# ReadAlongs/SoundSwallower

Hardware: AMD Instinct MI355X
Metric: senone-frames/sec (en-us PTM) (higher is better)
Workload: dtype f32+i32

## Files before the change

soundswallower_amd/csrc/ssw_k1a_mfma.inc:

```
typedef _Float16 f16x8 __attribute__((ext_vector_type(8)));
typedef _Float16 f16x2 __attribute__((ext_vector_type(2)));

#define SSW_MFMA_WIDEN 1.8537045e-05f
#define SSW_MFMA_XMAX 255.0f

typedef uint32_t u32x4 __attribute__((ext_vector_type(4)));

struct SplitX {
    f16x8 p[2];
};

__device__ __forceinline__ SplitX
split2_f16(const float (&v)[8])
{
    SplitX s;
    float r[8];
#pragma unroll
    for (int j = 0; j < 8; ++j)
        r[j] = v[j];
#pragma unroll
    for (int p = 0; p < 2; ++p) {
        u32x4 w;
#pragma unroll
        for (int j = 0; j < 8; j += 2) {
            const float2v pr = { r[j], r[j + 1] };
            const f16x2 h = __builtin_convertvector(pr, f16x2);
            w[j >> 1] = __builtin_bit_cast(uint32_t, h);
            if (p == 0) {
                asm("v_fma_mix_f32 %0, %1, -1.0, %2 op_sel_hi:[1,0,0]"
                    : "=v"(r[j]) : "v"(w[j >> 1]), "v"(r[j]));
                asm("v_fma_mix_f32 %0, %1, -1.0, %2 op_sel:[1,0,0] op_sel_hi:[1,0,0]"
                    : "=v"(r[j + 1]) : "v"(w[j >> 1]), "v"(r[j + 1]));
            }
        }
        s.p[p] = __builtin_bit_cast(f16x8, w);
    }
    return s;
}

struct XRaw {
    float4u a, b;
};

template <int VECLEN>
__device__ __forceinline__ XRaw
mfma_load_x(const float *__restrict__ xp, bool hi)
{
    static_assert(VECLEN == 13, "K layout: 13 dimensions, the constant at slot 15");
    XRaw r;
    r.a = *reinterpret_cast<const float4u *>(xp + (hi ? 8 : 0));
    r.b = *reinterpret_cast<const float4u *>(xp + (hi ? 9 : 4));
    return r;
}

__device__ __forceinline__ void
mfma_build_x(const XRaw &r, bool hi, float xconst, SplitX (&bx)[2])
{
    const float4u a = r.a, b = r.b;
    float v0[8], v1[8];
    v0[0] = a.x, v0[1] = a.y, v0[2] = a.z, v0[3] = a.w;
    v0[4] = hi ? b.w : b.x;
    v0[5] = hi ? 32768.0f : b.y;
    v0[6] = hi ? 32768.0f : b.z;
    v0[7] = hi ? xconst : b.w;
#pragma unroll
    for (int j = 0; j < 5; ++j)
        v1[j] = v0[j] * v0[j];
    v1[5] = hi ? 0.0f : b.y * b.y;
    v1[6] = hi ? 0.0f : b.z * b.z;
    v1[7] = hi ? 0.0f : b.w * b.w;
    bx[0] = split2_f16(v0);
    bx[1] = split2_f16(v1);
}

template <int VECLEN>
__device__ __forceinline__ void
mfma_build_x(const float *__restrict__ xp, bool hi, float xconst, SplitX (&bx)[2])
{
    mfma_build_x(mfma_load_x<VECLEN>(xp, hi), hi, xconst, bx);
}

__device__ __forceinline__ v16f
mfma_key_tile_frag(const f16x8 (&a)[2][2], const SplitX (&bx)[2])
{
    v16f acc = {};
#pragma unroll
    for (int kb = 0; kb < 2; ++kb) {
        acc = __builtin_amdgcn_mfma_f32_32x32x16_f16(a[kb][0], bx[kb].p[1], acc, 0, 0, 0);
        acc = __builtin_amdgcn_mfma_f32_32x32x16_f16(a[kb][1], bx[kb].p[0], acc, 0, 0, 0);
    }
#pragma unroll
    for (int kb = 0; kb < 2; ++kb)
        acc = __builtin_amdgcn_mfma_f32_32x32x16_f16(a[kb][0], bx[kb].p[0], acc, 0, 0, 0);
    return acc;
}

__device__ __forceinline__ v16f
mfma_key_tile(const uint4 *s_w, int rb, int lane, const SplitX (&bx)[2])
{
    f16x8 a[2][2];
#pragma unroll
    for (int kb = 0; kb < 2; ++kb)
#pragma unroll
        for (int p = 0; p < 2; ++p)
            a[kb][p] = __builtin_bit_cast(f16x8, s_w[((rb * 2 + kb) * 2 + p) * 64 + lane]);
    return mfma_key_tile_frag(a, bx);
}

template <int VECLEN>
__global__ void __launch_bounds__(64)
ptm_mfma_keys_kernel(const uint4 *__restrict__ wfrag, const float *__restrict__ recmax,
                     const float *__restrict__ feats, int n_frames, int featdim, int foff, int cbf,
                     float *__restrict__ out)
{
    const int lane = threadIdx.x & 63, col = lane & 31;
    const bool hi = lane >= 32;
    __shared__ uint4 s_w[16 * 64];
    for (int i = lane; i < 16 * 64; i += 64)
        s_w[i] = wfrag[(size_t)cbf * (16 * 64) + i];
    const float scale = recmax[(size_t)cbf * SSW_REC_FLOATS + 1];
    const float xconst = recmax[(size_t)cbf * SSW_REC_FLOATS + 3];
    __syncthreads();
    for (int cb = 0; cb < 4; ++cb) {
        const int t = (int)blockIdx.x * 128 + 32 * cb + col;
        const int tl = t < n_frames ? t : n_frames - 1;
        const float *xp = feats + (size_t)tl * featdim + foff;
        SplitX bx[2];
        mfma_build_x<VECLEN>(xp, hi, xconst, bx);
        for (int rb = 0; rb < 4; ++rb) {
            const v16f acc = mfma_key_tile(s_w, rb, lane, bx);
            if (t < n_frames)
#pragma unroll
                for (int r = 0; r < 16; ++r)
                    out[(size_t)t * 128 + 32 * rb + 8 * (r >> 2) + (hi ? 4 : 0) + (r & 3)]
                        = acc[r] * scale;
        }
    }
}

#define SSW_TOP5_INSERT(L, key) ssw_top5_insert(L, key);

__device__ __forceinline__ void
mfma_label_keys(const v16f &acc, int rb, uint32_t keymask, float (&key)[16])
{
#pragma unroll
    for (int r = 0; r < 16; ++r) {
        uint32_t lab;
        asm("s_add_i32 %0, %1, %2" : "=s"(lab) : "s"(16 * rb), "i"(r) : "scc");
        key[r] = __uint_as_float((__float_as_uint(acc[r]) & keymask) | lab);
    }
}

__device__ __forceinline__ void
mfma_swap_merge(float (&LA)[5], const float (&LB)[5], bool hi, float (&L)[5])
{
    const uint32_t half_bit = hi ? 64u : 0u;
#pragma unroll
    for (int k = 0; k < 5; ++k) {
        const float mine = hi ? LB[k] : LA[k], send = hi ? LA[k] : LB[k];
        const float got = __shfl_xor(__uint_as_float(__float_as_uint(send) | half_bit), 32, WAVE);
        L[k] = __uint_as_float(__float_as_uint(mine) | half_bit);
        LA[k] = got;
    }
#pragma unroll
    for (int k = 0; k < 5; ++k)
        SSW_TOP5_INSERT(L, LA[k])
}

__device__ __forceinline__ uint32_t
mfma_label_density(uint32_t lab)
{
    return ((lab >> 4) & 3u) * 32u + ((lab >> 2) & 3u) * 8u + (lab >> 6) * 4u + (lab & 3u);
}

#ifndef SSW_MFMA_WAVES
#define SSW_MFMA_WAVES 5
#endif
template <int VECLEN, bool MS, int NSTEP, bool AUDIT = false, bool MASKED = false>
__global__ void __launch_bounds__(256, SSW_MFMA_WAVES)
ptm_topn_mfma_kernel(const float *__restrict__ rec, const uint4 *__restrict__ wfrag,
                     const float *__restrict__ recmax, const uint32_t *__restrict__ exlist,
                     const float *__restrict__ feats, FramesParams P)
{
    static_assert(VECLEN == 13, "K layout: 13 dimensions, the constant at slot 15");
    const int lane = threadIdx.x & 63;
    const int col = lane & 31;
    const bool hi = lane >= 32;
    const int pair = P.xcd_lo[blockIdx.x & 7u] + (int)(blockIdx.x >> 3);
    if (pair >= P.xcd_lo[(blockIdx.x & 7u) + 1])
        return;
    const int cbf = pair / P.tile_groups;
    const int tile = (pair - cbf * P.tile_groups) * 4
        + __builtin_amdgcn_readfirstlane((int)(threadIdx.x >> 6));
    const int t_base = P.frame_lo + tile * (64 * NSTEP);
    const int f = cbf % P.n_feat;
    const int foff = P.featoff[f];

    __shared__ float4 s_rec[128 * (SSW_REC28_FLOATS / 4)];
    __shared__ uint4 s_w[16 * 64];
    uint2 ustart_v[NSTEP];
#pragma unroll
    for (int q = 0; q < NSTEP; ++q) {
        const int tq = t_base + 64 * q < P.n_frames ? t_base + 64 * q : 0;
        ustart_v[q] = *reinterpret_cast<const uint2 *>(P.utt_start + (tq >> 5));
    }
    const float4 cbc = *reinterpret_cast<const float4 *>(recmax + (size_t)cbf * SSW_REC_FLOATS);
    const float d0 = cbc.x, scale = cbc.y, inv_scale = cbc.z, xconst = cbc.w;
    static_assert(SSW_EXLIST_STRIDE >= 129, "two entries per lane behind the count");
    const uint32_t *xl = exlist + (size_t)cbf * SSW_EXLIST_STRIDE;
    const uint32_t n_ex_v = xl[0], my_ex0 = xl[1 + lane], my_ex1 = xl[65 + lane];
    int n_ex;
    constexpr bool pre_x = NSTEP == 1;
    SplitX bxa[2], bxb[2];
    auto x_row = [&](int t) {
        return feats + (size_t)(t < P.n_frames ? t : P.n_frames - 1) * P.featdim + foff;
    };
    {
        const float4 *src = reinterpret_cast<const float4 *>(rec + (size_t)cbf * 128 * SSW_REC28_FLOATS);
        const uint4 *wsrc = wfrag + (size_t)cbf * (16 * 64);
        uint4 wst[4];
        float4 stage[4];
#pragma unroll
        for (int i = 0; i < 4; ++i)
            stage[i] = src[i * 256 + (int)threadIdx.x < 896 ? i * 256 + (int)threadIdx.x : 895];
#pragma unroll
        for (int i = 0; i < 4; ++i)
            wst[i] = wsrc[i * 256 + (int)threadIdx.x];
        XRaw ra, rb;
        if (pre_x) {
            ra = mfma_load_x<VECLEN>(x_row(t_base + col), hi);
            rb = mfma_load_x<VECLEN>(x_row(t_base + 32 + col), hi);
        }
#pragma unroll
        for (int i = 0; i < 4; ++i) {
            const int e = i * 256 + (int)threadIdx.x;
            if (e < 896)
                s_rec[e] = stage[i];
        }
#pragma unroll
        for (int i = 0; i < 4; ++i)
            s_w[i * 256 + (int)threadIdx.x] = wst[i];
        if (pre_x) {
            mfma_build_x(ra, hi, xconst, bxa);
            mfma_build_x(rb, hi, xconst, bxb);
        }
        n_ex = __builtin_amdgcn_readfirstlane((int)n_ex_v);
    }
    unsigned long long ustart[NSTEP];
#pragma unroll
    for (int q = 0; q < NSTEP; ++q)
        ustart[q] = ((unsigned long long)(uint32_t)__builtin_amdgcn_readfirstlane((int)ustart_v[q].y) << 32)
            | (uint32_t)__builtin_amdgcn_readfirstlane((int)ustart_v[q].x);
    __syncthreads();
    if (t_base >= P.n_frames)
        return;
    SSW_TL(0)
#ifdef SSW_TIMELINE
    if (lane == 0) {
        int wv = blockIdx.x * 4 + (threadIdx.x >> 6);
        if (wv < 8192) {
            g_timeline[wv * 6 + 4] = __builtin_amdgcn_s_getreg(63492);
            g_timeline[wv * 6 + 5] = __builtin_amdgcn_s_getreg(20 | (31 << 11));
        }
    }
#endif

    uint32_t keymask;
    asm volatile("v_mov_b32 %0, 0xffffff80" : "=v"(keymask));
    const float NEG_INF = -__builtin_huge_valf();
    const float *srec_f = reinterpret_cast<const float *>(s_rec);

    uint32_t cpk[2] = { 0u, 0u };
    int s3[2] = { 0, 0 };
    unsigned long long need[2] = { 0ull, 0ull };
    unsigned long long audited[2] = { 0ull, 0ull };
    const bool audit_wave = AUDIT && P.audit_k > 0
        && (pair * 4 + __builtin_amdgcn_readfirstlane((int)(threadIdx.x >> 6))) % P.audit_k == 0;

#pragma unroll 1
    for (int step = 0; step < NSTEP; ++step) {
        const int t0 = t_base + 64 * step;
        if (!pre_x) {
            mfma_build_x<VECLEN>(x_row(t0 + col), hi, xconst, bxa);
            mfma_build_x<VECLEN>(x_row(t0 + 32 + col), hi, xconst, bxb);
        }
        float LA[5], LB[5], MA[2], MB[2], ZA, ZB;
        ssw_top5_reset(LA, MA, ZA, NEG_INF);
        ssw_top5_reset(LB, MB, ZB, NEG_INF);
#pragma unroll 1
        for (int rb = 0; rb < 4; ++rb) {
            f16x8 a[2][2];
#pragma unroll
            for (int kb = 0; kb < 2; ++kb)
#pragma unroll
                for (int p = 0; p < 2; ++p)
                    a[kb][p] = __builtin_bit_cast(f16x8, s_w[((rb * 2 + kb) * 2 + p) * 64 + lane]);
            {
                const v16f acc = mfma_key_tile_frag(a, bxa);
                float key[16];
                mfma_label_keys(acc, rb, keymask, key);
                ssw_top5_tile(LA, MA, ZA, key);
            }
            {
                const v16f acc = mfma_key_tile_frag(a, bxb);
                float key[16];
                mfma_label_keys(acc, rb, keymask, key);
                ssw_top5_tile(LB, MB, ZB, key);
            }
        }
        ssw_top5_fold(LA, MA, ZA);
        ssw_top5_fold(LB, MB, ZB);
        float L[5];
        mfma_swap_merge(LA, LB, hi, L);
        const int t = t0 + lane;
        const int tl = t < P.n_frames ? t : P.n_frames - 1;
        const float *xp = feats + (size_t)tl * P.featdim + foff;
        float x[VECLEN];
#pragma unroll
        for (int j = 0; j + 4 <= VECLEN; j += 4) {
            const float4u v = *reinterpret_cast<const float4u *>(xp + j);
            x[j] = v.x, x[j + 1] = v.y, x[j + 2] = v.z, x[j + 3] = v.w;
        }
#pragma unroll
        for (int j = VECLEN & ~3; j < VECLEN; ++j)
            x[j] = xp[j];
        float2v x2[6];
#pragma unroll
        for (int p = 0; p < 6; ++p)
            x2[p] = float2v{ x[2 * p], x[2 * p + 1] };
        auto exact_row = [&](uint32_t row) -> float {
            const unsigned char *rowp = reinterpret_cast<const unsigned char *>(s_rec)
                + row * (SSW_REC28_FLOATS * 4);
            float4v rv[SSW_REC28_FLOATS / 4];
#pragma unroll
            for (int q = 0; q < SSW_REC28_FLOATS / 4; ++q)
                rv[q] = *reinterpret_cast<const float4v *>(rowp + q * 16);
            asm volatile("" : "+v"(rv[0]), "+v"(rv[1]), "+v"(rv[2]), "+v"(rv[3]), "+v"(rv[4]),
                              "+v"(rv[5]), "+v"(rv[6]));
            float dd = rv[3].y;
#pragma unroll
            for (int p = 0; p < 6; ++p) {
                const float2v mean = (p & 1) ? float2v{ rv[p >> 1].z, rv[p >> 1].w }
                                             : float2v{ rv[p >> 1].x, rv[p >> 1].y };
                const int vq = (14 + 2 * p) >> 2;
                const float2v var = (p & 1) ? float2v{ rv[vq].x, rv[vq].y }
                                            : float2v{ rv[vq].z, rv[vq].w };
                const float2v diff = x2[p] - mean;
                const float2v sq = diff * diff;
                const float2v cc = sq * var;
                dd = dd - cc.x;
                dd = dd - cc.y;
            }
            {
                const float diff = x[12] - rv[3].x;
                const float sq = diff * diff;
                const float cc = sq * rv[6].z;
                dd = dd - cc;
            }
            return dd;
        };
        for (int i = 0; i < n_ex; ++i) {
            const int cwx = i < 64 ? __builtin_amdgcn_readlane((int)my_ex0, i)
                                   : __builtin_amdgcn_readlane((int)my_ex1, i - 64);
            float dd = exact_row((uint32_t)cwx);
            dd = (dd - d0) * inv_scale;
            const uint32_t lab = (uint32_t)((cwx & 3) | ((cwx >> 3) & 3) << 2 | (cwx >> 5) << 4
                                            | ((cwx >> 2) & 1) << 6);
            const float key = __uint_as_float((__float_as_uint(dd) & keymask) | lab);
            SSW_TOP5_INSERT(L, key)
        }
        int c[4], sk[4];
        float dv[4];
#pragma unroll
        for (int k = 0; k < 4; ++k) {
            const uint32_t lab = __float_as_uint(L[k]) & 127u;
            c[k] = (int)mfma_label_density(lab);
            dv[k] = exact_row((uint32_t)c[k]);
            sk[k] = MS ? ms_fden(dv[k]) : dens2int(dv[k]);
        }
#define CSWAP(a, b)                                                                          \
    {                                                                                        \
        bool sw_ = MS ? (dv[b] > dv[a]) : (sk[b] > sk[a]);                                   \
        int ts = sw_ ? sk[b] : sk[a], tc = sw_ ? c[b] : c[a];                                \
        float td = sw_ ? dv[b] : dv[a];                                                      \
        sk[b] = sw_ ? sk[a] : sk[b];                                                         \
        c[b] = sw_ ? c[a] : c[b];                                                            \
        dv[b] = sw_ ? dv[a] : dv[b];                                                         \
        sk[a] = ts;                                                                          \
        c[a] = tc;                                                                           \
        dv[a] = td;                                                                          \
    }
        CSWAP(0, 1) CSWAP(2, 3) CSWAP(0, 2) CSWAP(1, 3) CSWAP(1, 2)
#undef CSWAP
        uint32_t kb5 = __float_as_uint(L[4]);
        float ub = __uint_as_float((kb5 & 0x80000000u) ? (kb5 & ~127u) : (kb5 | 127u));
        ub = ub * scale;
        ub = ub + __builtin_fabsf(ub) * SSW_MFMA_WIDEN + 1.0e-3f;
        ub = ub + d0;
        ub = ub + __builtin_fabsf(ub) * 2.384185791015625e-07f;
        bool proven;
        if (MS)
            proven = dv[0] > dv[1] && dv[1] > dv[2] && dv[2] > dv[3] && dv[3] > ub;
        else
            proven = sk[0] > sk[1] && sk[1] > sk[2] && sk[2] > sk[3] && ub == ub
                && sk[3] > dens2int(ub);
        float am5;
        {
            float am0, am1, am2, am3, am4;
            asm("v_max3_f32 %0, |%1|, |%2|, |%3|" : "=v"(am0) : "v"(x[0]), "v"(x[1]), "v"(x[2]));
            asm("v_max3_f32 %0, |%1|, |%2|, |%3|" : "=v"(am1) : "v"(x[3]), "v"(x[4]), "v"(x[5]));
            asm("v_max3_f32 %0, |%1|, |%2|, |%3|" : "=v"(am2) : "v"(x[6]), "v"(x[7]), "v"(x[8]));
            asm("v_max3_f32 %0, |%1|, |%2|, |%3|" : "=v"(am3) : "v"(x[9]), "v"(x[10]), "v"(x[11]));
            asm("v_max3_f32 %0, %1, %2, |%3|" : "=v"(am4) : "v"(am0), "v"(am1), "v"(x[12]));
            asm("v_max3_f32 %0, %1, %2, %3" : "=v"(am5) : "v"(am2), "v"(am3), "v"(am4));
            proven = proven && am5 <= SSW_MFMA_XMAX;
        }
        const int floor_s = (L[3] > -4.0e9f && am5 <= SSW_MFMA_XMAX) ? sk[3] : INT_MIN;
        const uint32_t cpk_s = (uint32_t)c[0] | ((uint32_t)c[1] << 8) | ((uint32_t)c[2] << 16)
            | ((uint32_t)c[3] << 24);
        unsigned long long need_s = __ballot(!proven && t < P.n_frames);
        if (AUDIT && audit_wave) {
            const unsigned long long proven_s = __ballot(proven && t < P.n_frames);
            need_s |= proven_s;
#pragma unroll
            for (int q = 0; q < 2; ++q)
                audited[q] = q == step ? proven_s : audited[q];
        }
#pragma unroll
        for (int q = 0; q < 2; ++q) {
            cpk[q] = q == step ? cpk_s : cpk[q];
            s3[q] = q == step ? floor_s : s3[q];
            need[q] = q == step ? need_s : need[q];
        }
        if (t < P.n_frames) {
            const size_t idx = (size_t)t * P.n_cbf + cbf;
            P.topn_cw[idx] = cpk_s;
            P.topn_sc[idx] = make_int4(sk[0], sk[1], sk[2], sk[3]);
        }
        if (step == 0) {
            SSW_TL(1)
        }
    }
    SSW_TL(2)

    if (P.seg_of_frame != nullptr) {
#pragma unroll
        for (int q = 0; q < NSTEP; ++q) {
            const int tq = t_base + 64 * q + lane;
            need[q] &= __ballot(tq < P.n_frames
                                && cb_scanned(P, cbf / P.n_feat, tq < P.n_frames ? tq : 0));
            audited[q] &= need[q];
        }
    }
    if ((need[0] | (NSTEP > 1 ? need[1] : 0ull)) != 0ull) {
        const float *srow0 = srec_f + lane * SSW_REC28_FLOATS;
        const float *srow1 = srow0 + 64 * SSW_REC28_FLOATS;
        const int sw = 0;
        unsigned n_done = 0;
        SSW_TL2(0)
#pragma unroll
        for (int h = 0; h < NSTEP; ++h) {
            unsigned long long todo = need[h];
            while (todo != 0ull) {
                const int l = __builtin_ctzll(todo);
                todo &= todo - 1ull;
                const int t = t_base + 64 * h + l;
                float dvx[2];
                int ivx[2];
                wave_frame_densities<VECLEN, true, !MS>(feats, P.featdim, foff, t, srow0, srow1,
                                                        sw, dvx, ivx);
                if (n_done == 0) {
                    SSW_TL2(1)
                }
                int Lc[4], Ls[4];
                if (MS) {
                    float Ld[4];
                    ms_exact_step(dvx, Lc, Ld);
#pragma unroll
                    for (int k = 0; k < 4; ++k)
                        Ls[k] = ms_fden(Ld[k]);
                } else if (!topn_self_determined(ivx, lane, Lc, Ls)) {
                    if ((ustart[h] >> l) & 1ull) {
                        start_order(P, cbf, t, Lc);
                    } else if ((h == 0 && l == 0) || !cb_scanned_u(P, cbf / P.n_feat, t - 1)
                               || chain_skipped(P, t - 1)) {
                        carried_order_of<VECLEN, true, MASKED>(P, cbf, feats, foff, t - 1, lane, srow0,
                                                       srow1, sw, Lc);
                    } else {
                        const uint32_t pk = l == 0
                            ? (uint32_t)__builtin_amdgcn_readlane((int)cpk[0], 63)
                            : (uint32_t)__builtin_amdgcn_readlane((int)cpk[h], l - 1);
#pragma unroll
                        for (int k = 0; k < 4; ++k)
                            Lc[k] = (int)((pk >> (8 * k)) & 0xffu);
                    }
#pragma unroll
                    for (int k = 0; k < 4; ++k)
                        Ls[k] = INT_MIN;
                    topn_exact_step<2, 4>(dvx, ivx, Lc, Ls, true,
                                          __builtin_amdgcn_readlane(s3[h], l));
                }
                if (n_done == 0) {
                    SSW_TL2(2)
                }
                const bool was_proven = AUDIT && ((audited[h] >> l) & 1ull) != 0ull;
                if (AUDIT && was_proven) {
                    asm volatile("s_waitcnt vmcnt(0)" ::: "memory");
                    if (lane == l) {
                        const size_t idx = (size_t)t * P.n_cbf + cbf;
                        const uint32_t newpk = (uint32_t)Lc[0] | ((uint32_t)Lc[1] << 8)
                            | ((uint32_t)Lc[2] << 16) | ((uint32_t)Lc[3] << 24);
                        const int *old = reinterpret_cast<const int *>(P.topn_sc + idx);
                        bool same = __hip_atomic_load(P.topn_cw + idx, __ATOMIC_RELAXED,
                                                      __HIP_MEMORY_SCOPE_AGENT) == newpk;
#pragma unroll
                        for (int k = 0; k < 4; ++k)
                            same = same && __hip_atomic_load(old + k, __ATOMIC_RELAXED,
                                                             __HIP_MEMORY_SCOPE_AGENT) == Ls[k];
                        if (!same)
                            atomicAdd(P.n_fixed + 3, 1ull);
                    }
                }
                if (lane == l) {
                    cpk[h] = (uint32_t)Lc[0] | ((uint32_t)Lc[1] << 8) | ((uint32_t)Lc[2] << 16)
                        | ((uint32_t)Lc[3] << 24);
                    const size_t idx = (size_t)t * P.n_cbf + cbf;
                    P.topn_cw[idx] = cpk[h];
                    P.topn_sc[idx] = make_int4(Ls[0], Ls[1], Ls[2], Ls[3]);
                }
                if (!was_proven)
                    ++n_done;
            }
        }
        SSW_TL2(3)
#ifdef SSW_TIMELINE
        if (lane == 0) {
            int wv = blockIdx.x * 4 + (threadIdx.x >> 6);
            if (wv < 8192)
                g_timeline2[wv * 8 + 4] = n_done;
        }
#endif
        if (lane == 0)
            atomicAdd(P.n_fixed, (unsigned long long)n_done);
        if (AUDIT && lane == 0 && (audited[0] | audited[1]) != 0ull)
            atomicAdd(P.n_fixed + 2, (unsigned long long)(__builtin_popcountll(audited[0])
                                                          + __builtin_popcountll(audited[1])));
    }
    SSW_TL(3)
}
#undef SSW_TOP5_INSERT

__global__ void __launch_bounds__(64)
ptm_scan_top5_debug_kernel(const float *__restrict__ keys, int n_frames, int32_t *__restrict__ out_idx,
                           float *__restrict__ out_key)
{
    const int lane = threadIdx.x & 63, col = lane & 31;
    const bool hi = lane >= 32;
    const int t0 = (int)blockIdx.x * 64;
    uint32_t keymask;
    asm volatile("v_mov_b32 %0, 0xffffff80" : "=v"(keymask));
    const float NEG_INF = -__builtin_huge_valf();
    float LA[5], LB[5], MA[2], MB[2], ZA, ZB;
    ssw_top5_reset(LA, MA, ZA, NEG_INF);
    ssw_top5_reset(LB, MB, ZB, NEG_INF);
    auto tile_of = [&](int blk, int rb) {
        const int t = t0 + 32 * blk + col;
        const float *kp = keys + (size_t)(t < n_frames ? t : n_frames - 1) * 128 + 32 * rb
            + (hi ? 4 : 0);
        v16f acc;
#pragma unroll
        for (int r = 0; r < 16; ++r)
            acc[r] = kp[8 * (r >> 2) + (r & 3)];
        return acc;
    };
#pragma unroll 1
    for (int rb = 0; rb < 4; ++rb) {
        float key[16];
        mfma_label_keys(tile_of(0, rb), rb, keymask, key);
        ssw_top5_tile(LA, MA, ZA, key);
        mfma_label_keys(tile_of(1, rb), rb, keymask, key);
        ssw_top5_tile(LB, MB, ZB, key);
    }
    ssw_top5_fold(LA, MA, ZA);
    ssw_top5_fold(LB, MB, ZB);
    float L[5];
    mfma_swap_merge(LA, LB, hi, L);
    const int t = t0 + lane;
    if (t < n_frames)
#pragma unroll
        for (int k = 0; k < 5; ++k) {
            const uint32_t bits = __float_as_uint(L[k]);
            out_idx[(size_t)t * 5 + k] = (int32_t)mfma_label_density(bits & 127u);
            out_key[(size_t)t * 5 + k] = __uint_as_float(bits & ~127u);
        }
}

__global__ void __launch_bounds__(64)
mfma_f16_tile_kernel(const _Float16 *__restrict__ A, const _Float16 *__restrict__ B,
                     const float *__restrict__ C, float *__restrict__ D)
{
    const int l = threadIdx.x;
    const size_t tile = blockIdx.x;
    A += tile * 32 * 16, B += tile * 16 * 32, C += tile * 32 * 32, D += tile * 32 * 32;
    f16x8 a, b;
#pragma unroll
    for (int i = 0; i < 8; ++i) {
        a[i] = A[(l % 32) * 16 + 8 * (l / 32) + i];
        b[i] = B[(8 * (l / 32) + i) * 32 + (l % 32)];
    }
    v16f c;
#pragma unroll
    for (int r = 0; r < 16; ++r)
        c[r] = C[(8 * (r / 4) + 4 * (l / 32) + r % 4) * 32 + (l % 32)];
    const v16f d = __builtin_amdgcn_mfma_f32_32x32x16_f16(a, b, c, 0, 0, 0);
#pragma unroll
    for (int r = 0; r < 16; ++r)
        D[(8 * (r / 4) + 4 * (l / 32) + r % 4) * 32 + (l % 32)] = d[r];
}

__device__ __forceinline__ uint32_t
selftest_hash(uint32_t x)
{
    x ^= x >> 16; x *= 0x7feb352du; x ^= x >> 15; x *= 0x846ca68bu; x ^= x >> 16;
    return x;
}
__device__ __forceinline__ float
selftest_f16val(uint32_t h, int e_lo, int e_span)
{
    const int e = e_lo + (int)((h >> 11) % (uint32_t)e_span);
    const float v = (1.0f + (float)(h & 1023u) * (1.0f / 1024.0f)) * __builtin_exp2f((float)e);
    return (h >> 31) ? -v : v;
}

#define SSW_SELFTEST_ADVERSARIAL 24
#define SSW_SELFTEST_TILES (SSW_SELFTEST_ADVERSARIAL + 320)
__device__ float2 g_selftest_out[SSW_SELFTEST_TILES];
__global__ void __launch_bounds__(64)
mfma_selftest_kernel(uint32_t seed)
{
    float2 *out = g_selftest_out;
    const int l = threadIdx.x, col = l & 31, half = l >> 5;
    const uint32_t tile = blockIdx.x;
    float a[16], b[16];
    float cbig = 0.0f;
    int fam = -1;
    if (tile < SSW_SELFTEST_ADVERSARIAL) {
        const int j = tile >> 2;
        const bool above = (tile >> 1) & 1u, in_c = tile & 1u;
        const float frac = above ? 1.0f + 0.0009765625f : 1.0f - 0.00048828125f;
#pragma unroll
        for (int k = 0; k < 16; ++k) {
            a[k] = 0.03125f * frac;
            b[k] = __builtin_exp2f((float)(-6 - j));
        }
        if (in_c)
            cbig = 4096.0f;
        else
            a[0] = 64.0f, b[0] = 64.0f;
    } else {
        fam = (int)((tile - SSW_SELFTEST_ADVERSARIAL) % 5u);
#pragma unroll
        for (int k = 0; k < 16; ++k) {
            const uint32_t ha = selftest_hash(seed ^ (tile * 977u + (uint32_t)k * 131u + 1u));
            const uint32_t hb = selftest_hash(seed ^ (tile * 1409u + (uint32_t)k * 61u + (uint32_t)col * 7919u + 2u));
            if (fam == 2) {
                a[k] = selftest_f16val(ha, -10, 21);
                b[k] = selftest_f16val(hb, -10, 21);
            } else if (fam == 3) {
                a[k] = __builtin_fabsf(selftest_f16val(selftest_hash(seed ^ (tile * 977u)), -1, 2)) * ((k & 1) ? -1.0f : 1.0f);
                b[k] = __builtin_fabsf(selftest_f16val(selftest_hash(seed ^ (tile * 1409u + (uint32_t)col * 7919u)), -1, 2));
            } else {
                a[k] = selftest_f16val(ha, -2, 3);
                b[k] = selftest_f16val(hb, -2, 3);
            }
        }
        if (fam == 4)
            a[0] *= 4096.0f;
    }
    double dot = 0.0, terms = 0.0;
#pragma unroll
    for (int k = 0; k < 16; ++k) {
        const double pr = (double)a[k] * (double)b[k];
        dot += pr;
        terms += __builtin_fabs(pr);
    }
    f16x8 af, bf;
    v16f c;
    const float rs_own = fam < 0 ? 1.0f : __builtin_exp2f((float)((col % 3) - 1));
#pragma unroll
    for (int i = 0; i < 8; ++i) {
        af[i] = (_Float16)(a[8 * half + i] * rs_own);
        bf[i] = (_Float16)b[8 * half + i];
    }
    double cd[16], rs[16];
#pragma unroll
    for (int r = 0; r < 16; ++r) {
        const int row = 8 * (r / 4) + 4 * half + r % 4;
        rs[r] = fam < 0 ? 1.0 : (double)__builtin_exp2f((float)((row % 3) - 1));
        const uint32_t hc = selftest_hash(seed ^ (tile * 2741u + (uint32_t)row * 389u + (uint32_t)col * 17u + 3u));
        const float u01 = (float)(hc & 0xffffu) * (1.0f / 65536.0f);
        float cv;
        if (fam < 0)
            cv = cbig;
        else if (fam == 1 || fam == 3)
            cv = (float)(-(dot * rs[r]) * (1.0 + 1.0e-3 * (double)u01));
        else
            cv = (u01 - 0.5f) * (fam == 0 ? 1.0f : 8.0f);
        c[r] = cv;
        cd[r] = (double)cv;
    }
    const v16f d = __builtin_amdgcn_mfma_f32_32x32x16_f16(af, bf, c, 0, 0, 0);
    float worst = 0.0f;
#pragma unroll
    for (int r = 0; r < 16; ++r) {
        const double exact = dot * rs[r] + cd[r];
        const double tsum = terms * rs[r] + __builtin_fabs(cd[r]);
        const double err = __builtin_fabs((double)d[r] - exact);
        const float ratio = (float)(err / tsum * 16777216.0);
        worst = ratio > worst ? ratio : worst;
        if (!(d[r] == d[r]))
            worst = __builtin_huge_valf();
    }
#pragma unroll
    for (int off = 32; off >= 1; off >>= 1) {
        const float o = __shfl_xor(worst, off, WAVE);
        worst = o > worst ? o : worst;
    }
    if (l == 0)
        out[tile] = make_float2(worst, d[0]);
}
```

soundswallower_amd/csrc/ssw_top5_select.inc:

```
#ifndef SSW_SEL_FN
#define SSW_SEL_FN __device__ __forceinline__
SSW_SEL_FN float
ssw_sel_max2(float a, float b)
{
    float d;
    asm("v_max_f32 %0, %1, %2" : "=v"(d) : "v"(a), "v"(b));
    return d;
}
SSW_SEL_FN float
ssw_sel_max3(float a, float b, float c)
{
    float d;
    asm("v_max3_f32 %0, %1, %2, %3" : "=v"(d) : "v"(a), "v"(b), "v"(c));
    return d;
}
SSW_SEL_FN float
ssw_sel_min3(float a, float b, float c)
{
    float d;
    asm("v_min3_f32 %0, %1, %2, %3" : "=v"(d) : "v"(a), "v"(b), "v"(c));
    return d;
}
SSW_SEL_FN float
ssw_sel_med3(float a, float b, float c)
{
    return __builtin_amdgcn_fmed3f(a, b, c);
}
#endif

SSW_SEL_FN void
ssw_top5_insert(float (&H)[5], float key)
{
    H[4] = ssw_sel_med3(H[3], H[4], key);
    H[3] = ssw_sel_med3(H[2], H[3], key);
    H[2] = ssw_sel_med3(H[1], H[2], key);
    H[1] = ssw_sel_med3(H[0], H[1], key);
    H[0] = ssw_sel_max2(H[0], key);
}

SSW_SEL_FN void
ssw_top5_reset(float (&H)[5], float (&M)[2], float &Z, float neg_inf)
{
#pragma unroll
    for (int k = 0; k < 5; ++k)
        H[k] = neg_inf;
    M[0] = M[1] = Z = neg_inf;
}

SSW_SEL_FN void
ssw_top5_tile(float (&H)[5], float (&M)[2], float &Z, const float (&key)[16])
{
    float r3_held = 0.0f;
#pragma unroll
    for (int g = 0; g < 5; ++g) {
        const float a = key[3 * g], b = key[3 * g + 1], c = key[3 * g + 2];
        const float r1 = ssw_sel_max3(a, b, c);
        const float r2 = ssw_sel_med3(a, b, c);
        const float r3 = ssw_sel_min3(a, b, c);
        ssw_top5_insert(H, r1);
        M[1] = ssw_sel_med3(M[0], M[1], r2);
        M[0] = ssw_sel_max2(M[0], r2);
        if (g & 1)
            Z = ssw_sel_max3(Z, r3_held, r3);
        else if (g == 4)
            Z = ssw_sel_max2(Z, r3);
        else
            r3_held = r3;
    }
    ssw_top5_insert(H, key[15]);
}

SSW_SEL_FN void
ssw_top5_fold(float (&H)[5], const float (&M)[2], float Z)
{
    ssw_top5_insert(H, M[0]);
    ssw_top5_insert(H, M[1]);
    ssw_top5_insert(H, Z);
}
```

Before: 63.92 million.

## Hierarchize top-5 selection and merge wave halves with permlane32 swap

Adds a second tournament level to the per-tile top-5 selection. Group maxima are reduced in triples, so fewer full five-step inserts run per tile, and second and third runners-up are kept in side lists. The fold and final merge use position-bounded inserts that skip comparisons which cannot change the list, because of the known rank of each candidate. The cross-half exchange replaces two shuffles with the gfx950 permlane32_swap builtin, which cuts the extra work on that path. Correctness depends on the rank-bound arguments about where each candidate can land, and the change adds registers for the extra tracked values.

```diff
diff --git a/soundswallower_amd/csrc/ssw_k1a_mfma.inc b/soundswallower_amd/csrc/ssw_k1a_mfma.inc
--- a/soundswallower_amd/csrc/ssw_k1a_mfma.inc
+++ b/soundswallower_amd/csrc/ssw_k1a_mfma.inc
@@ -152,19 +152,16 @@
 }
 
 __device__ __forceinline__ void
-mfma_swap_merge(float (&LA)[5], const float (&LB)[5], bool hi, float (&L)[5])
-{
-    const uint32_t half_bit = hi ? 64u : 0u;
+mfma_swap_merge(float (&LA)[5], float (&LB)[5], float (&L)[5])
+{
 #pragma unroll
     for (int k = 0; k < 5; ++k) {
-        const float mine = hi ? LB[k] : LA[k], send = hi ? LA[k] : LB[k];
-        const float got = __shfl_xor(__uint_as_float(__float_as_uint(send) | half_bit), 32, WAVE);
-        L[k] = __uint_as_float(__float_as_uint(mine) | half_bit);
-        LA[k] = got;
-    }
-#pragma unroll
-    for (int k = 0; k < 5; ++k)
-        SSW_TOP5_INSERT(L, LA[k])
+        const auto sw = __builtin_amdgcn_permlane32_swap(__float_as_uint(LA[k]),
+                                                         __float_as_uint(LB[k]), false, false);
+        L[k] = __uint_as_float(sw[0]);
+        LB[k] = __uint_as_float(sw[1] | 64u);
+    }
+    ssw_top5_merge(L, LB);
 }
 
 __device__ __forceinline__ uint32_t
@@ -284,9 +281,9 @@
             mfma_build_x<VECLEN>(x_row(t0 + col), hi, xconst, bxa);
             mfma_build_x<VECLEN>(x_row(t0 + 32 + col), hi, xconst, bxb);
         }
-        float LA[5], LB[5], MA[2], MB[2], ZA, ZB;
-        ssw_top5_reset(LA, MA, ZA, NEG_INF);
-        ssw_top5_reset(LB, MB, ZB, NEG_INF);
+        float LA[5], LB[5], NA[2], NB[2], YA, YB, MA[2], MB[2], ZA, ZB;
+        ssw_top5_reset2(LA, NA, YA, MA, ZA, NEG_INF);
+        ssw_top5_reset2(LB, NB, YB, MB, ZB, NEG_INF);
 #pragma unroll 1
         for (int rb = 0; rb < 4; ++rb) {
             f16x8 a[2][2];
@@ -299,19 +296,19 @@
                 const v16f acc = mfma_key_tile_frag(a, bxa);
                 float key[16];
                 mfma_label_keys(acc, rb, keymask, key);
-                ssw_top5_tile(LA, MA, ZA, key);
+                ssw_top5_tile2(LA, NA, YA, MA, ZA, key);
             }
             {
                 const v16f acc = mfma_key_tile_frag(a, bxb);
                 float key[16];
                 mfma_label_keys(acc, rb, keymask, key);
-                ssw_top5_tile(LB, MB, ZB, key);
+                ssw_top5_tile2(LB, NB, YB, MB, ZB, key);
             }
         }
-        ssw_top5_fold(LA, MA, ZA);
-        ssw_top5_fold(LB, MB, ZB);
+        ssw_top5_fold2(LA, NA, YA, MA, ZA);
+        ssw_top5_fold2(LB, NB, YB, MB, ZB);
         float L[5];
-        mfma_swap_merge(LA, LB, hi, L);
+        mfma_swap_merge(LA, LB, L);
         const int t = t0 + lane;
         const int tl = t < P.n_frames ? t : P.n_frames - 1;
         const float *xp = feats + (size_t)tl * P.featdim + foff;
@@ -560,9 +557,9 @@
     uint32_t keymask;
     asm volatile("v_mov_b32 %0, 0xffffff80" : "=v"(keymask));
     const float NEG_INF = -__builtin_huge_valf();
-    float LA[5], LB[5], MA[2], MB[2], ZA, ZB;
-    ssw_top5_reset(LA, MA, ZA, NEG_INF);
-    ssw_top5_reset(LB, MB, ZB, NEG_INF);
+    float LA[5], LB[5], NA[2], NB[2], YA, YB, MA[2], MB[2], ZA, ZB;
+    ssw_top5_reset2(LA, NA, YA, MA, ZA, NEG_INF);
+    ssw_top5_reset2(LB, NB, YB, MB, ZB, NEG_INF);
     auto tile_of = [&](int blk, int rb) {
         const int t = t0 + 32 * blk + col;
         const float *kp = keys + (size_t)(t < n_frames ? t : n_frames - 1) * 128 + 32 * rb
@@ -577,14 +574,14 @@
     for (int rb = 0; rb < 4; ++rb) {
         float key[16];
         mfma_label_keys(tile_of(0, rb), rb, keymask, key);
-        ssw_top5_tile(LA, MA, ZA, key);
+        ssw_top5_tile2(LA, NA, YA, MA, ZA, key);
         mfma_label_keys(tile_of(1, rb), rb, keymask, key);
-        ssw_top5_tile(LB, MB, ZB, key);
-    }
-    ssw_top5_fold(LA, MA, ZA);
-    ssw_top5_fold(LB, MB, ZB);
+        ssw_top5_tile2(LB, NB, YB, MB, ZB, key);
+    }
+    ssw_top5_fold2(LA, NA, YA, MA, ZA);
+    ssw_top5_fold2(LB, NB, YB, MB, ZB);
     float L[5];
-    mfma_swap_merge(LA, LB, hi, L);
+    mfma_swap_merge(LA, LB, L);
     const int t = t0 + lane;
     if (t < n_frames)
 #pragma unroll
diff --git a/soundswallower_amd/csrc/ssw_top5_select.inc b/soundswallower_amd/csrc/ssw_top5_select.inc
--- a/soundswallower_amd/csrc/ssw_top5_select.inc
+++ b/soundswallower_amd/csrc/ssw_top5_select.inc
@@ -77,3 +77,80 @@
     ssw_top5_insert(H, M[1]);
     ssw_top5_insert(H, Z);
 }
+
+template <int FROM>
+SSW_SEL_FN void
+ssw_top5_insert_from(float (&H)[5], float key)
+{
+    static_assert(FROM >= 0 && FROM < 5, "a position of the list");
+#pragma unroll
+    for (int k = 4; k >= (FROM > 0 ? FROM : 1); --k)
+        H[k] = ssw_sel_med3(H[k - 1], H[k], key);
+    if (FROM == 0)
+        H[0] = ssw_sel_max2(H[0], key);
+}
+
+SSW_SEL_FN void
+ssw_top5_reset2(float (&H)[5], float (&N)[2], float &Y, float (&M)[2], float &Z, float neg_inf)
+{
+    ssw_top5_reset(H, M, Z, neg_inf);
+    N[0] = N[1] = Y = neg_inf;
+}
+
+SSW_SEL_FN void
+ssw_top5_tile2(float (&H)[5], float (&N)[2], float &Y, float (&M)[2], float &Z,
+               const float (&key)[16])
+{
+    float r1[6], r3_held = 0.0f, s3_held = 0.0f;
+#pragma unroll
+    for (int g = 0; g < 5; ++g) {
+        const float a = key[3 * g], b = key[3 * g + 1], c = key[3 * g + 2];
+        r1[g] = ssw_sel_max3(a, b, c);
+        const float r2 = ssw_sel_med3(a, b, c);
+        const float r3 = ssw_sel_min3(a, b, c);
+        M[1] = ssw_sel_med3(M[0], M[1], r2);
+        M[0] = ssw_sel_max2(M[0], r2);
+        if (g & 1)
+            Z = ssw_sel_max3(Z, r3_held, r3);
+        else if (g == 4)
+            Z = ssw_sel_max2(Z, r3);
+        else
+            r3_held = r3;
+    }
+    r1[5] = key[15];
+#pragma unroll
+    for (int g = 0; g < 2; ++g) {
+        const float a = r1[3 * g], b = r1[3 * g + 1], c = r1[3 * g + 2];
+        const float s1 = ssw_sel_max3(a, b, c);
+        const float s2 = ssw_sel_med3(a, b, c);
+        const float s3 = ssw_sel_min3(a, b, c);
+        ssw_top5_insert(H, s1);
+        N[1] = ssw_sel_med3(N[0], N[1], s2);
+        N[0] = ssw_sel_max2(N[0], s2);
+        if (g & 1)
+            Y = ssw_sel_max3(Y, s3_held, s3);
+        else
+            s3_held = s3;
+    }
+}
+
+SSW_SEL_FN void
+ssw_top5_fold2(float (&H)[5], const float (&N)[2], float Y, const float (&M)[2], float Z)
+{
+    ssw_top5_insert_from<1>(H, N[0]);
+    ssw_top5_insert_from<3>(H, N[1]);
+    ssw_top5_insert_from<2>(H, Y);
+    ssw_top5_insert_from<1>(H, M[0]);
+    ssw_top5_insert_from<3>(H, M[1]);
+    ssw_top5_insert_from<2>(H, Z);
+}
+
+SSW_SEL_FN void
+ssw_top5_merge(float (&H)[5], const float (&G)[5])
+{
+    ssw_top5_insert_from<0>(H, G[0]);
+    ssw_top5_insert_from<1>(H, G[1]);
+    ssw_top5_insert_from<2>(H, G[2]);
+    ssw_top5_insert_from<3>(H, G[3]);
+    ssw_top5_insert_from<4>(H, G[4]);
+}
```

After: 64.94 million, median of 6. +1.6%, better.
